# LongmaoTeamTf/deep_recommenders

Hardware: AMD Instinct MI355X
Metric: examples/sec/node DeepFM (26 sparse feats, 10M vocab, dim 64) (higher is better)
Workload: dtype f32; 1 GPU; DeepFM Criteo-shape synthetic training step (BASELINE.json configs[2]): 26 sparse + 13 dense, 10000000 vocab/field hashed on device, dim 64, DNN [256, 32]+[1] relu, sigmoid-CE, fused SGD; batch 65536 per GPU, ids uniform; tables on one GPU (66.6 GB); gemm_split=f16x2, global_batch=65536, parallelism=single, per_kernel_events=False

## Files before the change

deep_recommenders_amd/csrc/bf3_wgrad.hip:

```cpp
#ifndef DR_NT_WGRAD_GATHER
#define DR_NT_WGRAD_GATHER 0
#endif
#include "bf3_rs_core.h"

namespace {

using namespace drrs;

struct TnRsArgs {
    const float* X; int64_t ldx;
    const float* Y; int64_t ldy;
    int64_t R; int32_t F; int32_t N;
    int64_t per; int32_t split;
    float* partial; float* colsum;
    const int32_t* ids_t; const int64_t* row_base; const float* table; int32_t nf; const float* dense_pad;
    const uint32_t* x_amax; const uint32_t* x2_amax; const uint32_t* y_amax;
};

template <int GATHER, int H2 = 0>
__global__ __launch_bounds__(512, 2) void bf3_gemm_tn_rs_kernel(TnRsArgs g) {
    constexpr int NW = 8, BMF = 32 * NW, BN = 256, NT = BN / 32;
    constexpr int NPL = RS_NPL<H2>, B_PLANE = RS_B_PLANE, STAGE = RS_STAGE<H2>;
    __shared__ __attribute__((aligned(1024))) unsigned char smem[2 * STAGE];

    const int tid = threadIdx.x, lane = tid & 63;
    const int wave = __builtin_amdgcn_readfirstlane(tid >> 6);
    const int l31 = lane & 31, hi = lane >> 5;
    const int tiles_n = (g.N + BN - 1) / BN, tiles_f = (g.F + BMF - 1) / BMF;
    const int per_slice = tiles_f * tiles_n;
    const int Fp = tiles_f * BMF, Np = tiles_n * BN;
    const int lid = xcd_remap(blockIdx.x, per_slice * g.split);
    const int slice = lid / per_slice, t = lid % per_slice;
    const int f0 = (t / tiles_n) * BMF, n0 = (t % tiles_n) * BN;
    const int64_t r_begin = (int64_t)slice * g.per;
    int64_t r_end = r_begin + g.per;
    if (r_end > g.R) r_end = g.R;
    const int nk = (int)((r_end - r_begin + BK - 1) / BK);
    const bool want_cs = g.colsum != nullptr && f0 == 0;
    float h2_sx = 1.f, h2_sy = 1.f;
    if constexpr (H2) {
        float inv;
        h2_prologue(g.x_amax, g.x2_amax, g.y_amax, h2_sx, h2_sy, inv);
    }

    const int fcol = min(f0 + wave * 32 + l31, g.F - 1);
    const int ncol = min(n0 + wave * 32 + l31, g.N - 1);
    const unsigned lds0 = (unsigned)(uintptr_t)(lds_ptr_t)smem;
    const int sw = tn_img_swizzle(l31);
    unsigned b_addr[2];
#pragma unroll
    for (int s = 0; s < 2; ++s) b_addr[s] = rs_frag_addr(lds0, l31, hi, sw, s);
    unsigned char* const wrow = smem + (wave * 32 + l31) * 64;

    float xa[16], yb[16];
    const unsigned xoff = (unsigned)((16 * hi * g.ldx + fcol) * 4), yoff = (unsigned)((16 * hi * g.ldy + ncol) * 4);
    auto load_raw = [&](float (&dst)[16], const float* base, int64_t ld, unsigned voff, int64_t r0) {
        if (r0 + BK <= r_end) {
// ... 156 lines not shown
            __builtin_amdgcn_sched_barrier(0);
        }
    }
    float* out = g.partial + ((int64_t)slice * Fp + f0 + wave * 32 + 4 * hi) * Np + n0 + l31;
#pragma unroll
    for (int nt = 0; nt < NT; ++nt)
#pragma unroll
        for (int reg = 0; reg < 16; ++reg) out[(int64_t)((reg & 3) + 8 * (reg >> 2)) * Np + nt * 32] = acc[nt][reg];
    if (want_cs) {
        cs += __shfl_xor(cs, 32, 64);
        if (hi == 0) g.colsum[(int64_t)slice * Np + n0 + wave * 32 + l31] = cs;
    }
}

template <int V>
__global__ __launch_bounds__(64) void bf3_tn_rs_reduce_kernel(const float* __restrict__ partial, const float* __restrict__ colsum,
                                                              int32_t split, int32_t F, int32_t N, int32_t Fp, int32_t Np,
                                                              float scale, float* __restrict__ dst, int64_t ld,
                                                              float* __restrict__ dstb, const uint32_t* __restrict__ x_amax = nullptr,
                                                              const uint32_t* __restrict__ x2_amax = nullptr,
                                                              const uint32_t* __restrict__ y_amax = nullptr) {
    typedef float vec_t __attribute__((ext_vector_type(V)));
    const int f = blockIdx.x;
    const int n = ((int)blockIdx.y * 64 + (int)threadIdx.x) * V;
    if (n >= N) return;
    const int64_t ps = (int64_t)Fp * Np;
    float wscale = scale;
    if (x_amax != nullptr) {
        float sx, ix, sy, iy;
        h2_scale_of(max(x_amax[0], x2_amax != nullptr ? x2_amax[0] : 0u), sx, ix);
        h2_scale_of(y_amax[0], sy, iy);
        wscale = scale * (ix * iy);
    }
    auto sum_slices = [&](const float* p, int64_t stride) -> vec_t {
        vec_t acc = 0.f;
        int s = 0;
        for (; s + 8 <= split; s += 8) {
            vec_t v[8];
#pragma unroll
            for (int u = 0; u < 8; ++u) v[u] = *reinterpret_cast<const vec_t*>(p + (s + u) * stride);
#pragma unroll
            for (int u = 0; u < 8; ++u) acc += v[u];
        }
        for (; s < split; ++s) acc += *reinterpret_cast<const vec_t*>(p + s * stride);
        return acc;
    };
    const vec_t acc = sum_slices(partial + (int64_t)f * Np + n, ps);
    float* d = dst + (int64_t)f * ld + n;
    if (V == 1 || n + V <= N) {
        vec_t o = *reinterpret_cast<vec_t*>(d);
#pragma unroll
        for (int c = 0; c < V; ++c) o[c] = fmaf(wscale, acc[c], o[c]);
        *reinterpret_cast<vec_t*>(d) = o;
    } else {
#pragma unroll
        for (int c = 0; c < V; ++c)
            if (n + c < N) d[c] = fmaf(wscale, acc[c], d[c]);
    }
    if (f == 0 && colsum != nullptr && dstb != nullptr) {
        const vec_t cacc = sum_slices(colsum + n, Np);
#pragma unroll
        for (int c = 0; c < V; ++c)
            if (n + c < N) dstb[n + c] = fmaf(scale, cacc[c], dstb[n + c]);
    }
}

void launch_tn_rs_reduce(const float* partial, const float* colsum, int split, int32_t F, int32_t N, int Fp, int Np, float scale,
                         float* dst, int64_t ld, float* dstb, const uint32_t* x_amax, const uint32_t* x2_amax, const uint32_t* y_amax,
                         dr_stream_t stream) {
    const bool vec = ((reinterpret_cast<uintptr_t>(partial) | reinterpret_cast<uintptr_t>(dst)) & 15) == 0 && (ld & 3) == 0;
    if (vec)
        hipLaunchKernelGGL(bf3_tn_rs_reduce_kernel<4>, dim3(F, (N + 255) / 256), dim3(64), 0, dr_s(stream), partial, colsum, split, F, N,
                           Fp, Np, scale, dst, ld, dstb, x_amax, x2_amax, y_amax);
    else
        hipLaunchKernelGGL(bf3_tn_rs_reduce_kernel<1>, dim3(F, (N + 63) / 64), dim3(64), 0, dr_s(stream), partial, colsum, split, F, N,
                           Fp, Np, scale, dst, ld, dstb, x_amax, x2_amax, y_amax);
}

void tn_rs_plan(int64_t R, int32_t F, int32_t N, int& split, int64_t& per, int& Fp, int& Np) {
    const int tf = (F + 255) / 256, tn = (N + 255) / 256;
    Fp = tf * 256;
    Np = tn * 256;
    int64_t sp = 256 / ((int64_t)tf * tn);
    const int64_t max_split = (R + 16 * BK - 1) / (16 * BK);
    if (sp > max_split) sp = max_split;
    if (sp < 1) sp = 1;
    per = ((R + sp - 1) / sp + BK - 1) / BK * BK;
    split = (int)((R + per - 1) / per);
}
}

extern "C" int64_t dr_bf3_wgrad_workspace_bytes(int64_t R, int32_t F, int32_t N) {
    if (R <= 0 || F <= 0 || N <= 0) return 0;
    int split, Fp, Np;
    int64_t per;
    tn_rs_plan(R, F, N, split, per, Fp, Np);
    return ((int64_t)split * Fp * Np + (int64_t)split * Np) * (int64_t)sizeof(float);
}

static int wgrad_impl(const float* x, int64_t ld_x, const float* dy, int64_t ld_dy, int64_t R, int32_t F, int32_t N,
                      float scale, float* dstW, int64_t ld_w, float* dstb, void* workspace, int64_t workspace_bytes,
                      dr_stream_t stream, const uint32_t* x_amax = nullptr, const uint32_t* dy_amax = nullptr) {
    if (R <= 0 || F <= 0 || N <= 0) return DR_EINVAL;
    if (!x || !dy || !dstW || !workspace || ld_x < F || ld_dy < N || ld_w < N) return DR_EINVAL;
    if (workspace_bytes < dr_bf3_wgrad_workspace_bytes(R, F, N)) return DR_EINVAL;
    int split, Fp, Np;
    int64_t per;
    tn_rs_plan(R, F, N, split, per, Fp, Np);
    float* partial = static_cast<float*>(workspace);
    float* colsum = partial + (int64_t)split * Fp * Np;
    TnRsArgs g{x, ld_x, dy, ld_dy, R, F, N, per, split, partial, dstb != nullptr ? colsum : nullptr, nullptr, nullptr, nullptr, 0, nullptr,
               x_amax, nullptr, dy_amax};
    const int grid = (Fp / 256) * (Np / 256) * split;
    if (x_amax != nullptr) hipLaunchKernelGGL((bf3_gemm_tn_rs_kernel<0, 1>), dim3(grid), dim3(512), 0, dr_s(stream), g);
    else hipLaunchKernelGGL((bf3_gemm_tn_rs_kernel<0, 0>), dim3(grid), dim3(512), 0, dr_s(stream), g);
    launch_tn_rs_reduce(partial, dstb != nullptr ? colsum : nullptr, split, F, N, Fp, Np, scale, dstW, ld_w, dstb, x_amax, nullptr, dy_amax,
                        stream);
    DR_CHECK_LAUNCH();
    return DR_OK;
}

extern "C" int dr_bf3_wgrad(const float* x, int64_t ld_x, const float* dy, int64_t ld_dy, int64_t R, int32_t F, int32_t N,
                            float scale, float* dstW, int64_t ld_w, float* dstb, void* workspace, int64_t workspace_bytes,
                            dr_stream_t stream) {
    return wgrad_impl(x, ld_x, dy, ld_dy, R, F, N, scale, dstW, ld_w, dstb, workspace, workspace_bytes, stream);
}

extern "C" int dr_h2_wgrad(const float* x, int64_t ld_x, const uint32_t* x_amax, const float* dy, int64_t ld_dy, const uint32_t* dy_amax,
                           int64_t R, int32_t F, int32_t N, float scale, float* dstW, int64_t ld_w, float* dstb, void* workspace,
                           int64_t workspace_bytes, dr_stream_t stream) {
    if (!x_amax || !dy_amax) return DR_EINVAL;
    return wgrad_impl(x, ld_x, dy, ld_dy, R, F, N, scale, dstW, ld_w, dstb, workspace, workspace_bytes, stream, x_amax, dy_amax);
}

static int wgrad_emb_impl(const int32_t* ids_t, int64_t R, int32_t nf, const int64_t* row_base, const float* table, int32_t D,
                          const float* dense_pad, const float* dy, int64_t ld_dy, int32_t F, int32_t N, float scale, float* dstW,
                          int64_t ld_w, float* dstb, void* workspace, int64_t workspace_bytes, int32_t parts, dr_stream_t stream,
                          const uint32_t* table_amax = nullptr, const uint32_t* dense_amax = nullptr, const uint32_t* dy_amax = nullptr) {
    if (R <= 0 || F <= 0 || N <= 0 || nf <= 0) return DR_EINVAL;
    if (table_amax != nullptr && (!dy_amax || (F > 64 * nf && !dense_amax))) return DR_EINVAL;
    if (D != 64 || F < 64 * nf || F > 64 * nf + 32) return DR_ESHAPE;
    if (!ids_t || !row_base || !table || !dy || !dstW || !workspace || ld_dy < N || ld_w < N) return DR_EINVAL;
    if (F > 64 * nf && !dense_pad) return DR_EINVAL;
    if (workspace_bytes < dr_bf3_wgrad_workspace_bytes(R, F, N)) return DR_EINVAL;
    int split, Fp, Np;
    int64_t per;
    tn_rs_plan(R, F, N, split, per, Fp, Np);
    float* partial = static_cast<float*>(workspace);
    float* colsum = partial + (int64_t)split * Fp * Np;
    TnRsArgs g{nullptr, 0, dy, ld_dy, R, F, N, per, split, partial, dstb != nullptr ? colsum : nullptr, ids_t, row_base, table, nf,
               F > 64 * nf ? dense_pad : nullptr, table_amax, F > 64 * nf ? dense_amax : nullptr, dy_amax};
    const int grid = (Fp / 256) * (Np / 256) * split;
    if (parts & 1) {
        if (table_amax != nullptr) hipLaunchKernelGGL((bf3_gemm_tn_rs_kernel<1, 1>), dim3(grid), dim3(512), 0, dr_s(stream), g);
        else hipLaunchKernelGGL((bf3_gemm_tn_rs_kernel<1, 0>), dim3(grid), dim3(512), 0, dr_s(stream), g);
    }
    if (parts & 2)
        launch_tn_rs_reduce(partial, dstb != nullptr ? colsum : nullptr, split, F, N, Fp, Np, scale, dstW, ld_w, dstb, table_amax,
                            F > 64 * nf ? dense_amax : nullptr, dy_amax, stream);
    DR_CHECK_LAUNCH();
    return DR_OK;
}

extern "C" int dr_bf3_wgrad_emb(const int32_t* ids_t, int64_t R, int32_t nf, const int64_t* row_base, const float* table, int32_t D,
                                const float* dense_pad, const float* dy, int64_t ld_dy, int32_t F, int32_t N, float scale, float* dstW,
                                int64_t ld_w, float* dstb, void* workspace, int64_t workspace_bytes, int32_t parts, dr_stream_t stream) {
    if (parts < 1 || parts > 3) return DR_EINVAL;
    return wgrad_emb_impl(ids_t, R, nf, row_base, table, D, dense_pad, dy, ld_dy, F, N, scale, dstW, ld_w, dstb, workspace, workspace_bytes,
                          parts, stream);
}

extern "C" int dr_h2_wgrad_emb(const int32_t* ids_t, int64_t R, int32_t nf, const int64_t* row_base, const float* table, int32_t D,
                               const uint32_t* table_amax, const float* dense_pad, const uint32_t* dense_amax, const float* dy, int64_t ld_dy,
                               const uint32_t* dy_amax, int32_t F, int32_t N, float scale, float* dstW, int64_t ld_w, float* dstb,
// ... 6 lines not shown
```

deep_recommenders_amd/csrc/emb_sorted.hip:

```cpp
#include <cstdlib>
#include "dr_common.h"
#include <hip/amd_detail/amd_hip_unsafe_atomics.h>
#include <cstring>

namespace {

constexpr int CH = 32;

#ifndef DR_K4_NT
#define DR_K4_NT 1
#endif
typedef float dr_f4v __attribute__((ext_vector_type(4)));
__device__ __forceinline__ float4 ld4_stream(const float* p) {
#if DR_K4_NT
    const dr_f4v v = __builtin_nontemporal_load(reinterpret_cast<const dr_f4v*>(p));
    return make_float4(v.x, v.y, v.z, v.w);
#else
    return *reinterpret_cast<const float4*>(p);
#endif
}
__device__ __forceinline__ void st4_stream(float* p, const float4 v) {
#if DR_K4_NT
    const dr_f4v w = {v.x, v.y, v.z, v.w};
    __builtin_nontemporal_store(w, reinterpret_cast<dr_f4v*>(p));
// ... 309 lines not shown
template <int LPR, int U, bool ADAM>
__global__ DR_K4_LB void emb_bwd_sorted_kernel(BwdSortedArgs a, AdamArgs ad, int grid_d) {
    if ((int)blockIdx.x < grid_d)
        emb_bwd_dups_body<LPR, ADAM>(blockIdx.x, grid_d, a.rows, a.slots, a.n, a.dup_heads, a.dup_count, a.F, a.D, a.num_rows, a.grad,
                                     a.ld, a.concat, a.ldc, a.sum_x, a.d_fm_logit, a.slot_lin, a.scale, a.table, a.lin_w, ad, a.x_sorted,
                                     a.det != 0, a.amax);
    else if (a.dups_only) {
        if (!ADAM && a.lin_bias != nullptr && a.d_fm_logit != nullptr) dr_block_sum_axpy(a.d_fm_logit, a.B, a.scale, a.lin_bias);
    } else
        emb_bwd_unique_body<LPR, U, ADAM>(blockIdx.x - grid_d, gridDim.x - grid_d, a.ids, a.flags, a.B, a.F, a.row_base, a.D, a.grad,
                                          a.ld, a.concat, a.ldc, a.sum_x, a.d_fm_logit, a.slot_lin, a.scale, a.table,
                                          a.skip_unique_lin ? nullptr : a.lin_w, a.lin_bias, ad, a.lin_old_t, a.amax);
}

template <int LPR>
__global__ __launch_bounds__(256) void emb_bwd_hot_apply_kernel(BwdSortedArgs a) {
    constexpr int NS = DR_WAVE / LPR;
    const int lane = threadIdx.x & 63, grp = lane / LPR, sub = lane % LPR;
    const int D = a.D, F = a.F;
    const bool dvalid = sub < (D >> 2);
    const int subc = dvalid ? sub : (D >> 2) - 1;
    const bool any_lin = a.lin_w != nullptr && (a.d_fm_logit != nullptr || a.slot_lin != nullptr);
    const int64_t nwaves = (int64_t)gridDim.x * (blockDim.x >> 6);
    const int64_t wave0 = (int64_t)blockIdx.x * (blockDim.x >> 6) + (threadIdx.x >> 6);
    const int64_t nheads = a.dup_count[0], n = a.dup_count[1];
    float wmax = 0.f;
    constexpr int SCREEN = 16;
    for (int64_t h0 = wave0 * SCREEN; h0 < nheads; h0 += nwaves * SCREEN) {
        const int64_t h = h0 + lane;
        int64_t my_i = 0, my_stop = 0;
// ... 74 lines not shown
                if (lane == 0) a.lin_w[k] = fmaf(a.scale, dls, a.lin_w[k]);
            }
        }
    }
    if (a.amax != nullptr) amax_commit(a.amax, wmax);
}

}

static int bwd_sorted_impl(const int64_t* ids, const int64_t* row_base, const int64_t* sorted_rows,
                           const int32_t* sorted_slots, const uint8_t* unique_flags, const int32_t* dup_heads,
                           const int32_t* dup_count, int64_t B, int32_t F, int32_t D, int64_t num_rows, const float* grad,
                           int64_t ld_grad, const float* concat, int64_t ld_concat, const float* sum_x,
                           const float* d_fm_logit, const float* slot_lin_grad, float scale, float* dst_table,
                           float* dst_lin, float* dst_bias, const AdamArgs* adam, float* x_sorted, dr_stream_t stream,
                           int parts, const float* lin_old_t, uint32_t* table_amax) {
    if (B < 0 || F <= 0 || F > 64 || D < 4 || D > 256 || (D & 3) || num_rows <= 0) return DR_EINVAL;
    const int64_t n = B * F;
    if (n == 0) return DR_OK;
    if (!ids || !row_base || !sorted_rows || !sorted_slots || !unique_flags || !dup_heads || !dup_count || !grad ||
        !dst_table ||
        ld_grad < (int64_t)F * D || (ld_grad & 3))
        return DR_EINVAL;
    if (concat != nullptr && (ld_concat < (int64_t)F * D || (ld_concat & 3) || sum_x == nullptr)) return DR_EINVAL;
    if (sum_x != nullptr && d_fm_logit == nullptr) return DR_EINVAL;
    if (sum_x != nullptr && concat == nullptr && x_sorted == nullptr) return DR_EINVAL;
    int lpr = 1;
    while (lpr * 4 < D) lpr <<= 1;
    const uint64_t* rows = reinterpret_cast<const uint64_t*>(sorted_rows);
    const int grid_u = dr_grid_for(B, 4, 8192);
    const int grid_d = 2048;
    AdamArgs ad{};
    if (adam != nullptr) ad = *adam;
    static const bool det_on = [] { const char* e = getenv("DR_K4_DETERMINISTIC"); return !(e != nullptr && e[0] == '0'); }();
    const int det = (adam == nullptr && x_sorted != nullptr && det_on) ? 1 : 0;
    const BwdSortedArgs ba{ids, unique_flags, B, F, row_base, D, grad, ld_grad, concat, ld_concat, sum_x, d_fm_logit, slot_lin_grad,
                           scale, dst_table, dst_lin, dst_bias, rows, sorted_slots, n, dup_heads, dup_count, (uint64_t)num_rows,
                           x_sorted, det, (adam == nullptr && (parts & 4)) ? 1 : 0,
                           slot_lin_grad == nullptr ? lin_old_t : nullptr, table_amax, (parts & 8) ? 1 : 0};
#ifdef DR_K4_U
    constexpr int K4_U_OVERRIDE = DR_K4_U;
#else
    constexpr int K4_U_OVERRIDE = 0;
#endif
#define LAUNCH(L, ADAM_)                                                                                              \
    {                                                                                                                 \
        constexpr int NS_ = 64 / L;                                                                                   \
        constexpr int U_ = K4_U_OVERRIDE > 0 ? K4_U_OVERRIDE : (NS_ >= 16 ? 2 : 4);                                   \
        hipLaunchKernelGGL((emb_bwd_sorted_kernel<L, U_, ADAM_>), dim3(grid_d + ((parts & 8) ? 1 : grid_u)), dim3(256), 0, dr_s(stream), ba, ad,    \
                           grid_d);                                                                                   \
    }
#define CALL(L)                                                                                                       \
    if (adam != nullptr) LAUNCH(L, true) else LAUNCH(L, false)
    if (parts & 1)
    switch (lpr) {
        case 1: CALL(1); break;
        case 2: CALL(2); break;
        case 4: CALL(4); break;
        case 8: CALL(8); break;
        case 16: CALL(16); break;
        case 32: CALL(32); break;
        case 64: CALL(64); break;
        default: return DR_EINVAL;
    }
#undef CALL
#undef LAUNCH
// ... 15 lines not shown
    return DR_OK;
}

extern "C" int dr_emb_pool_bwd_sorted(const int64_t* ids, const int64_t* row_base, const int64_t* sorted_rows,
                                      const int32_t* sorted_slots, const uint8_t* unique_flags,
                                      const int32_t* dup_heads, const int32_t* dup_count, int64_t B, int32_t F,
                                      int32_t D, int64_t num_rows, const float* grad, int64_t ld_grad,
                                      const float* concat, int64_t ld_concat, const float* sum_x,
                                      const float* d_fm_logit, const float* slot_lin_grad, float scale,
                                      float* dst_table, float* dst_lin, float* dst_bias, float* x_sorted,
                                      const float* lin_old_t, int32_t parts, uint32_t* table_amax, dr_stream_t stream) {
    if (parts < 1 || parts > 15 || (parts & 3) == 0) return DR_EINVAL;
    return bwd_sorted_impl(ids, row_base, sorted_rows, sorted_slots, unique_flags, dup_heads, dup_count, B, F, D, num_rows,
                           grad, ld_grad, concat, ld_concat, sum_x, d_fm_logit, slot_lin_grad, scale, dst_table, dst_lin,
                           dst_bias, nullptr, x_sorted, stream, parts, lin_old_t, table_amax);
}

namespace {
__global__ __launch_bounds__(256) void lin_update_unique_kernel(const int64_t* __restrict__ ids, const uint8_t* __restrict__ flags,
                                                                int64_t n, int32_t F, const int64_t* __restrict__ row_base,
                                                                const float* __restrict__ d_fm_logit,
                                                                const float* __restrict__ slot_lin, float scale,
                                                                float* __restrict__ lin_w) {
    const int64_t stride = (int64_t)gridDim.x * blockDim.x;
    for (int64_t s = (int64_t)blockIdx.x * blockDim.x + threadIdx.x; s < n; s += stride) {
        const int64_t id = ids[s];
        if (id < 0 || !flags[s]) continue;
        const int64_t b = s / F;
        const int f = (int)(s - b * F);
        const int64_t row = row_base[f] + id;
// ... 215 lines not shown
```

deep_recommenders_amd/engine.py:

```python
import math
import os
from typing import List, Optional, Sequence

import torch

from . import ops
from .ops import _pad4


_SIDE_STREAMS = {}


def _side_streams(device):
    key = str(torch.device(device))
    if key not in _SIDE_STREAMS:
        _SIDE_STREAMS[key] = (torch.cuda.Stream(device=device), torch.cuda.Stream(device=device))
    return _SIDE_STREAMS[key]


class DeepFMEngine:
    def __init__(self, num_fields: int, vocab_per_field: int, dim: int, dnn_units: Sequence[int], batch: int,
                 num_dense: int = 0, lr: float = 0.01, device="cuda", seed: int = 42, hashed: bool = True,
                 table_init_std: Optional[float] = None, lin_init_std: float = 0.0, sorted_bwd: bool = True,
                 optimizer: str = "sgd", beta1: float = 0.9, beta2: float = 0.999, eps: float = 1e-8):
# ... 154 lines not shown
                        and D == 64 and not self.lin_side and self.lin_old_t is not None
                        and self.Ws[0].shape[0] >= F * D)
        _rs = os.environ.get("DR_REDUCE_SIDE", "0")
        self.reduce_side = sorted_bwd and optimizer == "sgd" and _rs in ("1", "2")
        self.reduce_side_wgrad = self.reduce_side and _rs == "1" and not self.h2
        self._small_pending = False
        self._planes_pending = False
        self._planes_pending_l0 = False
        self._k4_fused_done = False
        self._in_train_step = False
        self._early_issued = False
        _ov = os.environ.get("DR_OVERLAP_DW", "0")
        self.overlap_dw = _ov == "1"
        if self.overlap_dw:
            self.no_concat = False
        self.concurrent = {}
        if self.overlap_dw:
            k4 = "emb_pool_bwd_adam" if optimizer == "adam" else "emb_pool_bwd"
            self.concurrent = {"linear_bwd_dw_L0": k4, k4: "linear_bwd_dw_L0"}
            self.side2 = torch.cuda.Stream(device=device)
            self.ev_dx = torch.cuda.Event()
            self.ev_dw = torch.cuda.Event()

    @property
    def dense_pad(self):
        return self._dense_pads[self.cur] if self._dense_pads is not None else None

    @property
    def dense_amax(self):
        return self._dense_amaxs[self.cur] if self._dense_amaxs is not None else None
# ... 143 lines not shown
                tot += max(first.elapsed_time(fa), first.elapsed_time(fb))
            out.append({"kernels": [a, b], "joint_us": tot / n * 1e3})
        return out

    def _wgrad_reduce_deferred(self, i):
        return self.reduce_side_wgrad and i == 0 and self.no_concat and self.wplanes[0] is not None and not self.overlap_dw

    def _side_part2(self, fn):
        self.ev_part1.record()
        with torch.cuda.stream(self.side):
            self.side.wait_event(self.ev_part1)
            fn()
            self.ev_small.record(self.side)
        self._small_pending = True

    def _wgrad(self, i, x, dy, sc, dstW, dstb):
        if i == 0 and self.h2:
            ops.h2_wgrad_emb(self._ids_t[self.cur], self.row_base, self.table, self.tab_amax, self.dense_pad, self.dense_amax, dy,
                             self.dh0_amax, sc, dstW, dstb, workspace=self.wg_ws[0], parts=1 if self._wgrad_reduce_deferred(i) else 3)
        elif i == 0 and self.no_concat:
            ops.bf3_wgrad_emb(self._ids_t[self.cur], self.row_base, self.table, self.dense_pad, dy, sc, dstW, dstb,
                              workspace=self.wg_ws[0], parts=1 if self._wgrad_reduce_deferred(i) else 3)
        elif self.wg_ws[i] is not None:
            ops.bf3_wgrad(x, dy, sc, dstW, dstb, workspace=self.wg_ws[i])
        else:
            ops.linear_bwd_dw(x, dy, sc, dstW, dstb, workspace=self.dw_ws[i])

    def forward(self, keys: torch.Tensor, dense: Optional[torch.Tensor], labels: Optional[torch.Tensor],
                loss_mode: int = ops.LOSS_SIGMOID_CE):
        F, D = self.F, self.D
        B = self.B
        if self.optimizer == "adam":
            self.flat_grads.zero_()
        if self._planes_pending:
# ... 258 lines not shown
                torch.cuda.current_stream().wait_event(self.ev_lin)
            self._prefetch_issue(mark)
        else:
            self._k("emb_pool_bwd", "hbm", self.alg_bytes_bwd(),
                    lambda: ops.emb_pool_bwd(self.ids, F, self.col_start, self.row_base, D, self.d_concat, self.concat,
                                             self.sum_x, self.d_logit, -lr, self.table, self.lin_w, self.lin_bias))
        if self._small_pending:
            torch.cuda.current_stream().wait_event(self.ev_small)
            self._small_pending = False
        if self.overlap_dw and not adam:
            torch.cuda.current_stream().wait_event(self.ev_dw)

    def _backward_l0_fused_k4(self, x, dy, sc, dstW, dstb, fl):
        lr = self.lr
        torch.cuda.current_stream().wait_event(self.ev_sorted)
        self._k("linear_bwd_dw_L0", "mfma", fl, lambda: self._wgrad(0, x, dy, sc, dstW, dstb))
        w_old = self.wplanes[0].w
        early = self._early_issued
        rs = self.side_r if early else self.side
        self._refresh_stream = rs
        self.ev_dw_done.record()
        with torch.cuda.stream(rs):
            rs.wait_event(self.ev_dw_done)
            self.wplanes[0].refresh()
            self.ev_planes.record(rs)
        self._planes_pending = True
        self._planes_pending_l0 = True
        mark = self._prefetch_mark()
        if early:
            self._prefetch_issue(mark)
        if not self._k4_det:
            ops.emb_snapshot_sorted_rows(self.plan, self.table, self.R, self.x_sorted)
        work = self.alg_bytes_bwd() - 4.0 * self.B * self.F * self.D + 4.0 * self.B * dy.shape[1]
        self._k("emb_pool_bwd_fused_dgrad_L0", "hbm", work,
                lambda: ops.h2_dgrad_emb_sgd(dy, self.dh0_amax, w_old, self._ids_t[self.cur], self.plan, self.row_base, self.table,
                                             self.lin_w, self.lin_old_t, self.sum_x, self.d_logit, -lr, self.d_concat, table_amax=self.tab_amax))
        k4 = lambda parts: ops.emb_pool_bwd_sorted(self.ids, self.row_base, self.plan, self.D, self.R, self.d_concat, self.d_logit, -lr,
                                                   self.table, self.lin_w, self.lin_bias, sum_x=self.sum_x, x_sorted=self.x_sorted,
                                                   parts=parts | 8, lin_old_t=self.lin_old_t, table_amax=self.tab_amax)
        self._k("emb_pool_bwd_dups", "hbm", 0, lambda: k4(1))
        self._k("emb_hot_rows_apply", "hbm", 0, lambda: k4(2))
        if not early:
            self._prefetch_issue(mark)
        self._k4_fused_done = True

    def _launch_sort(self):
        self.ev_ids.record()
        with torch.cuda.stream(self.side):
            self.side.wait_event(self.ev_ids)
            self._k("emb_sort_slots(side stream, overlapped)", "overlap", self.B * self.F * 36,
                    lambda: ops.emb_sort_slots(self.ids, self.row_base, self.R, self.plan))
            self.ev_sorted.record(self.side)

    def _adam_finish(self):
        self.t += 1
# ... 78 lines not shown
```

deep_recommenders_amd/ops.py:

```python
from typing import Optional, Sequence

import torch

from . import _lib
from ._lib import check, lib, ptr, stream_ptr


def _c(t: torch.Tensor, dtype) -> torch.Tensor:
    if t.dtype != dtype:
        raise TypeError("expected %s, got %s" % (dtype, t.dtype))
    return t if t.is_contiguous() else t.contiguous()


def hash_bucket_i64(keys: torch.Tensor, col_buckets: torch.Tensor, out: Optional[torch.Tensor] = None):
    keys = _c(keys, torch.int64)
    B, C = keys.shape
    col_buckets = _c(col_buckets, torch.int64)
    assert col_buckets.numel() == C
    if out is None:
        out = torch.empty_like(keys)
    check(lib().dr_hash_bucket_i64(ptr(keys), B, C, ptr(col_buckets), ptr(out), stream_ptr()), "dr_hash_bucket_i64")
    return out


# ... 533 lines not shown
    return out


def emb_pool_bwd_sorted(ids, row_base, plan, D, num_rows, grad, d_fm_logit, scale, dst_table, dst_lin=None, dst_bias=None,
                        concat=None, sum_x=None, slot_lin_grad=None, x_sorted=None, parts=3, lin_old_t=None, table_amax=None):
    ids = _c(ids, torch.int64)
    B, F = ids.shape
    assert grad.stride(1) == 1
    assert lin_old_t is None or (lin_old_t.shape == (F, B) and lin_old_t.is_contiguous() and lin_old_t.dtype == torch.float32)
    check(lib().dr_emb_pool_bwd_sorted(ptr(ids), ptr(row_base), ptr(plan.rows), ptr(plan.slots), ptr(plan.flags),
                                       ptr(plan.dup_heads), ptr(plan.dup_count), B, F, D, int(num_rows), ptr(grad),
                                       grad.stride(0), ptr(concat), concat.stride(0) if concat is not None else 0,
                                       ptr(sum_x), ptr(d_fm_logit), ptr(slot_lin_grad), float(scale), ptr(dst_table), ptr(dst_lin),
                                       ptr(dst_bias), ptr(x_sorted), ptr(lin_old_t), int(parts), ptr(table_amax), stream_ptr()),
          "dr_emb_pool_bwd_sorted")


def h2_dgrad_emb_sgd(dy, dy_amax, w: "H2Planes", ids_t, plan, row_base, table, lin_w, lin_old_t, sum_x, d_fm_logit, scale, d_concat,
                     table_amax=None):
    F, M = ids_t.shape
    K = dy.shape[1]
    assert dy.stride(1) == 1 and d_concat.stride(1) == 1 and table.is_contiguous() and table.shape[1] == 64 and sum_x.is_contiguous()
    assert ids_t.dtype == torch.int32 and ids_t.is_contiguous() and dy.shape[0] == M and w.rows >= 64 * F
    assert (lin_w is None) == (lin_old_t is None)
    assert lin_old_t is None or (lin_old_t.shape == (F, M) and lin_old_t.is_contiguous())
    check(lib().dr_h2_dgrad_emb_sgd(ptr(dy), dy.stride(0), ptr(dy_amax), ptr(w.buf), w.plane_stride, w.ld, ptr(w.amax), M, F, K,
                                    ptr(ids_t), ptr(plan.flags), ptr(row_base), ptr(table), ptr(lin_w), ptr(lin_old_t), ptr(sum_x),
                                    ptr(d_fm_logit), float(scale), ptr(d_concat), d_concat.stride(0), ptr(table_amax), stream_ptr()),
          "dr_h2_dgrad_emb_sgd")

# ... 2217 lines not shown
```

include/dr_hotpath.h:

```cpp
#ifndef DR_HOTPATH_H
#define DR_HOTPATH_H

#include <stdint.h>

#ifdef __cplusplus
extern "C" {
#endif

#define DR_OK 0
#define DR_EINVAL (-1)
#define DR_ELAUNCH (-2)
#define DR_ESHAPE (-3)

typedef void* dr_stream_t;

const char* dr_version(void);

#define DR_GEMM_BF16X3 0
#define DR_GEMM_NATIVE_F32 1
int32_t dr_set_gemm_mode(int32_t mode);
int32_t dr_get_gemm_mode(void);

#define DR_GEMM_SPLIT_BF16X3 0
#define DR_GEMM_SPLIT_F16X2 1
// ... 277 lines not shown
                              const float* dense_pad, const uint32_t* dense_amax, float* concat, int64_t ld_concat, int32_t K,
                              const void* wt_planes, int64_t plane_stride, int64_t ld_planes, const uint32_t* w_amax, int32_t N,
                              const float* bias, int32_t act, float* sum_x, float* fm_logit, float* out, int64_t ld_out,
                              float* lin_vals_t, const float* W1, int64_t ld_w1, const float* b1, int32_t H, const float* w2,
                              int64_t ld_w2, const float* b2, const float* labels, int32_t loss_mode, float scale, float* dst_w1,
                              int64_t ld_dst_w1, float* dst_b1, float* dst_w2, int64_t ld_dst_w2, float* dst_b2, float* prob,
                              float* d_logit, float* d_h, int64_t ld_dh, float* dx, int64_t ld_dx, float* loss_out, void* workspace,
                              int64_t workspace_bytes, int32_t parts, uint32_t* dx_amax, dr_stream_t stream);
int dr_h2_wgrad(const float* x, int64_t ld_x, const uint32_t* x_amax, const float* dy, int64_t ld_dy, const uint32_t* dy_amax, int64_t R,
                int32_t F, int32_t N, float scale, float* dstW, int64_t ld_w, float* dstb, void* workspace, int64_t workspace_bytes,
                dr_stream_t stream);
int dr_h2_wgrad_emb(const int32_t* ids_t, int64_t R, int32_t nf, const int64_t* row_base, const float* table, int32_t D,
                    const uint32_t* table_amax, const float* dense_pad, const uint32_t* dense_amax, const float* dy, int64_t ld_dy,
                    const uint32_t* dy_amax, int32_t F, int32_t N, float scale, float* dstW, int64_t ld_w, float* dstb, void* workspace,
                    int64_t workspace_bytes, int32_t parts, dr_stream_t stream);


int dr_cin_fwd(const float* x0, const float* x, int64_t B, int32_t H0, int32_t Hk, int32_t D, const float* W,
               int32_t Fm, const float* bias, int32_t act, float* out, dr_stream_t stream);
int dr_cin_bwd(const float* x0, const float* x, int64_t B, int32_t H0, int32_t Hk, int32_t D, const float* W,
               int32_t Fm, int32_t act, const float* out, const float* d_out, float* d_x0, float* d_x, float* dW,
               float* dbias, dr_stream_t stream);

int dr_cin_pool_fwd(const float* x0, const float* x, int64_t B, int32_t H0, int32_t Hk, int32_t D, const float* W, int32_t Fm,
                    const float* bias, int32_t act, float* out, float* pooled, dr_stream_t stream);
int64_t dr_cin_pool_bwd_workspace_bytes(int64_t B, int32_t H0, int32_t Hk, int32_t D, int32_t Fm);
int dr_cin_pool_bwd(const float* x0, const float* x, int64_t B, int32_t H0, int32_t Hk, int32_t D, const float* W, int32_t Fm,
                    int32_t act, const float* out, const float* d_out, const float* d_pooled, float* d_x0, int32_t accumulate_x0,
                    float* d_x, float* dW, float* dbias, void* ws, int64_t ws_bytes, dr_stream_t stream);

// ... 176 lines not shown
```

Measured before the change: 70.79 million examples/sec.

## Fold wgrad split-K reduce into embedding dups backward kernel as rider blocks

The layer-0 weight-gradient split-K reduction no longer runs as its own kernel. It is appended as extra rider blocks to the embedding duplicate-row backward kernel, which removes a launch and lets the two memory-bound phases overlap. The GEMM kernel now writes the amax scale values into a workspace header, so the reduce no longer depends on amax buffers that the embedding update may mutate. The plane refresh is moved to after the fused kernel. This adds coupling and raises the risk of ordering bugs between the table amax update and the reduce scaling.

```diff
diff --git a/deep_recommenders_amd/csrc/bf3_wgrad.hip b/deep_recommenders_amd/csrc/bf3_wgrad.hip
--- a/deep_recommenders_amd/csrc/bf3_wgrad.hip
+++ b/deep_recommenders_amd/csrc/bf3_wgrad.hip
@@ -2,6 +2,7 @@
 #define DR_NT_WGRAD_GATHER 0
 #endif
 #include "bf3_rs_core.h"
+#include "tn_rs_reduce.h"
 
 namespace {
 
@@ -15,6 +16,7 @@
     float* partial; float* colsum;
     const int32_t* ids_t; const int64_t* row_base; const float* table; int32_t nf; const float* dense_pad;
     const uint32_t* x_amax; const uint32_t* x2_amax; const uint32_t* y_amax;
+    uint32_t* hdr;
 };
 
 template <int GATHER, int H2 = 0>
@@ -41,6 +43,10 @@
     if constexpr (H2) {
         float inv;
         h2_prologue(g.x_amax, g.x2_amax, g.y_amax, h2_sx, h2_sy, inv);
+        if (lid == 0 && tid == 0) {
+            g.hdr[0] = max(g.x_amax[0], g.x2_amax != nullptr ? g.x2_amax[0] : 0u);
+            g.hdr[1] = g.y_amax[0];
+        }
     }
 
     const int fcol = min(f0 + wave * 32 + l31, g.F - 1);
@@ -227,70 +233,18 @@
 }
 
 template <int V>
-__global__ __launch_bounds__(64) void bf3_tn_rs_reduce_kernel(const float* __restrict__ partial, const float* __restrict__ colsum,
-                                                              int32_t split, int32_t F, int32_t N, int32_t Fp, int32_t Np,
-                                                              float scale, float* __restrict__ dst, int64_t ld,
-                                                              float* __restrict__ dstb, const uint32_t* __restrict__ x_amax = nullptr,
-                                                              const uint32_t* __restrict__ x2_amax = nullptr,
-                                                              const uint32_t* __restrict__ y_amax = nullptr) {
-    typedef float vec_t __attribute__((ext_vector_type(V)));
-    const int f = blockIdx.x;
-    const int n = ((int)blockIdx.y * 64 + (int)threadIdx.x) * V;
-    if (n >= N) return;
-    const int64_t ps = (int64_t)Fp * Np;
-    float wscale = scale;
-    if (x_amax != nullptr) {
-        float sx, ix, sy, iy;
-        h2_scale_of(max(x_amax[0], x2_amax != nullptr ? x2_amax[0] : 0u), sx, ix);
-        h2_scale_of(y_amax[0], sy, iy);
-        wscale = scale * (ix * iy);
-    }
-    auto sum_slices = [&](const float* p, int64_t stride) -> vec_t {
-        vec_t acc = 0.f;
-        int s = 0;
-        for (; s + 8 <= split; s += 8) {
-            vec_t v[8];
-#pragma unroll
-            for (int u = 0; u < 8; ++u) v[u] = *reinterpret_cast<const vec_t*>(p + (s + u) * stride);
-#pragma unroll
-            for (int u = 0; u < 8; ++u) acc += v[u];
-        }
-        for (; s < split; ++s) acc += *reinterpret_cast<const vec_t*>(p + s * stride);
-        return acc;
-    };
-    const vec_t acc = sum_slices(partial + (int64_t)f * Np + n, ps);
-    float* d = dst + (int64_t)f * ld + n;
-    if (V == 1 || n + V <= N) {
-        vec_t o = *reinterpret_cast<vec_t*>(d);
-#pragma unroll
-        for (int c = 0; c < V; ++c) o[c] = fmaf(wscale, acc[c], o[c]);
-        *reinterpret_cast<vec_t*>(d) = o;
-    } else {
-#pragma unroll
-        for (int c = 0; c < V; ++c)
-            if (n + c < N) d[c] = fmaf(wscale, acc[c], d[c]);
-    }
-    if (f == 0 && colsum != nullptr && dstb != nullptr) {
-        const vec_t cacc = sum_slices(colsum + n, Np);
-#pragma unroll
-        for (int c = 0; c < V; ++c)
-            if (n + c < N) dstb[n + c] = fmaf(scale, cacc[c], dstb[n + c]);
-    }
-}
-
-void launch_tn_rs_reduce(const float* partial, const float* colsum, int split, int32_t F, int32_t N, int Fp, int Np, float scale,
-                         float* dst, int64_t ld, float* dstb, const uint32_t* x_amax, const uint32_t* x2_amax, const uint32_t* y_amax,
-                         dr_stream_t stream) {
-    const bool vec = ((reinterpret_cast<uintptr_t>(partial) | reinterpret_cast<uintptr_t>(dst)) & 15) == 0 && (ld & 3) == 0;
-    if (vec)
-        hipLaunchKernelGGL(bf3_tn_rs_reduce_kernel<4>, dim3(F, (N + 255) / 256), dim3(64), 0, dr_s(stream), partial, colsum, split, F, N,
-                           Fp, Np, scale, dst, ld, dstb, x_amax, x2_amax, y_amax);
-    else
-        hipLaunchKernelGGL(bf3_tn_rs_reduce_kernel<1>, dim3(F, (N + 63) / 64), dim3(64), 0, dr_s(stream), partial, colsum, split, F, N,
-                           Fp, Np, scale, dst, ld, dstb, x_amax, x2_amax, y_amax);
-}
-
-void tn_rs_plan(int64_t R, int32_t F, int32_t N, int& split, int64_t& per, int& Fp, int& Np) {
+__global__ __launch_bounds__(TN_RS_RED_THREADS) void bf3_tn_rs_reduce_kernel(TnRsApply a) {
+    tn_rs_reduce_block<V>(a, blockIdx.x, threadIdx.x);
+}
+
+void launch_tn_rs_reduce(const TnRsApply& a, dr_stream_t stream) {
+    const int nlb = tn_rs_reduce_blocks(a.F, a.N, a.vec);
+    if (a.vec) hipLaunchKernelGGL(bf3_tn_rs_reduce_kernel<4>, dim3(nlb), dim3(TN_RS_RED_THREADS), 0, dr_s(stream), a);
+    else hipLaunchKernelGGL(bf3_tn_rs_reduce_kernel<1>, dim3(nlb), dim3(TN_RS_RED_THREADS), 0, dr_s(stream), a);
+}
+}
+
+void drrs::tn_rs_plan(int64_t R, int32_t F, int32_t N, int& split, int64_t& per, int& Fp, int& Np) {
     const int tf = (F + 255) / 256, tn = (N + 255) / 256;
     Fp = tf * 256;
     Np = tn * 256;
@@ -301,14 +255,13 @@
     per = ((R + sp - 1) / sp + BK - 1) / BK * BK;
     split = (int)((R + per - 1) / per);
 }
-}
 
 extern "C" int64_t dr_bf3_wgrad_workspace_bytes(int64_t R, int32_t F, int32_t N) {
     if (R <= 0 || F <= 0 || N <= 0) return 0;
     int split, Fp, Np;
     int64_t per;
     tn_rs_plan(R, F, N, split, per, Fp, Np);
-    return ((int64_t)split * Fp * Np + (int64_t)split * Np) * (int64_t)sizeof(float);
+    return ((int64_t)split * Fp * Np + (int64_t)split * Np + TN_RS_HDR_WORDS) * (int64_t)sizeof(float);
 }
 
 static int wgrad_impl(const float* x, int64_t ld_x, const float* dy, int64_t ld_dy, int64_t R, int32_t F, int32_t N,
@@ -320,15 +273,14 @@
     int split, Fp, Np;
     int64_t per;
     tn_rs_plan(R, F, N, split, per, Fp, Np);
-    float* partial = static_cast<float*>(workspace);
-    float* colsum = partial + (int64_t)split * Fp * Np;
-    TnRsArgs g{x, ld_x, dy, ld_dy, R, F, N, per, split, partial, dstb != nullptr ? colsum : nullptr, nullptr, nullptr, nullptr, 0, nullptr,
-               x_amax, nullptr, dy_amax};
+    const bool h2 = x_amax != nullptr;
+    const TnRsApply ap = tn_rs_apply_of(workspace, split, F, N, Fp, Np, h2, scale, dstW, ld_w, dstb);
+    TnRsArgs g{x, ld_x, dy, ld_dy, R, F, N, per, split, const_cast<float*>(ap.partial), const_cast<float*>(ap.colsum), nullptr, nullptr, nullptr, 0,
+               nullptr, x_amax, nullptr, dy_amax, const_cast<uint32_t*>(ap.hdr)};
     const int grid = (Fp / 256) * (Np / 256) * split;
-    if (x_amax != nullptr) hipLaunchKernelGGL((bf3_gemm_tn_rs_kernel<0, 1>), dim3(grid), dim3(512), 0, dr_s(stream), g);
+    if (h2) hipLaunchKernelGGL((bf3_gemm_tn_rs_kernel<0, 1>), dim3(grid), dim3(512), 0, dr_s(stream), g);
     else hipLaunchKernelGGL((bf3_gemm_tn_rs_kernel<0, 0>), dim3(grid), dim3(512), 0, dr_s(stream), g);
-    launch_tn_rs_reduce(partial, dstb != nullptr ? colsum : nullptr, split, F, N, Fp, Np, scale, dstW, ld_w, dstb, x_amax, nullptr, dy_amax,
-                        stream);
+    launch_tn_rs_reduce(ap, stream);
     DR_CHECK_LAUNCH();
     return DR_OK;
 }
@@ -359,18 +311,16 @@
     int split, Fp, Np;
     int64_t per;
     tn_rs_plan(R, F, N, split, per, Fp, Np);
-    float* partial = static_cast<float*>(workspace);
-    float* colsum = partial + (int64_t)split * Fp * Np;
-    TnRsArgs g{nullptr, 0, dy, ld_dy, R, F, N, per, split, partial, dstb != nullptr ? colsum : nullptr, ids_t, row_base, table, nf,
-               F > 64 * nf ? dense_pad : nullptr, table_amax, F > 64 * nf ? dense_amax : nullptr, dy_amax};
+    const bool h2 = table_amax != nullptr;
+    const TnRsApply ap = tn_rs_apply_of(workspace, split, F, N, Fp, Np, h2, scale, dstW, ld_w, dstb);
+    TnRsArgs g{nullptr, 0, dy, ld_dy, R, F, N, per, split, const_cast<float*>(ap.partial), const_cast<float*>(ap.colsum), ids_t, row_base, table,
+               nf, F > 64 * nf ? dense_pad : nullptr, table_amax, F > 64 * nf ? dense_amax : nullptr, dy_amax, const_cast<uint32_t*>(ap.hdr)};
     const int grid = (Fp / 256) * (Np / 256) * split;
     if (parts & 1) {
-        if (table_amax != nullptr) hipLaunchKernelGGL((bf3_gemm_tn_rs_kernel<1, 1>), dim3(grid), dim3(512), 0, dr_s(stream), g);
+        if (h2) hipLaunchKernelGGL((bf3_gemm_tn_rs_kernel<1, 1>), dim3(grid), dim3(512), 0, dr_s(stream), g);
         else hipLaunchKernelGGL((bf3_gemm_tn_rs_kernel<1, 0>), dim3(grid), dim3(512), 0, dr_s(stream), g);
     }
-    if (parts & 2)
-        launch_tn_rs_reduce(partial, dstb != nullptr ? colsum : nullptr, split, F, N, Fp, Np, scale, dstW, ld_w, dstb, table_amax,
-                            F > 64 * nf ? dense_amax : nullptr, dy_amax, stream);
+    if (parts & 2) launch_tn_rs_reduce(ap, stream);
     DR_CHECK_LAUNCH();
     return DR_OK;
 }
diff --git a/deep_recommenders_amd/csrc/emb_sorted.hip b/deep_recommenders_amd/csrc/emb_sorted.hip
--- a/deep_recommenders_amd/csrc/emb_sorted.hip
+++ b/deep_recommenders_amd/csrc/emb_sorted.hip
@@ -1,5 +1,6 @@
 #include <cstdlib>
 #include "dr_common.h"
+#include "tn_rs_reduce.h"
 #include <hip/amd_detail/amd_hip_unsafe_atomics.h>
 #include <cstring>
 
@@ -347,6 +348,19 @@
 }
 
 template <int LPR>
+__global__ __launch_bounds__(256) void emb_bwd_dups_apply_kernel(BwdSortedArgs a, drrs::TnRsApply ap, int grid_d) {
+    const int bid = blockIdx.x;
+    if (bid < grid_d)
+        emb_bwd_dups_body<LPR, false>(bid, grid_d, a.rows, a.slots, a.n, a.dup_heads, a.dup_count, a.F, a.D, a.num_rows, a.grad, a.ld,
+                                      a.concat, a.ldc, a.sum_x, a.d_fm_logit, a.slot_lin, a.scale, a.table, a.lin_w, AdamArgs{}, a.x_sorted,
+                                      a.det != 0, a.amax);
+    else if (bid == grid_d) {
+        if (a.lin_bias != nullptr && a.d_fm_logit != nullptr) dr_block_sum_axpy(a.d_fm_logit, a.B, a.scale, a.lin_bias);
+    } else
+        drrs::tn_rs_reduce_ride(ap, bid - grid_d - 1, (int)gridDim.x - grid_d - 1, threadIdx.x);
+}
+
+template <int LPR>
 __global__ __launch_bounds__(256) void emb_bwd_hot_apply_kernel(BwdSortedArgs a) {
     constexpr int NS = DR_WAVE / LPR;
     const int lane = threadIdx.x & 63, grp = lane / LPR, sub = lane % LPR;
@@ -451,7 +465,7 @@
                            int64_t ld_grad, const float* concat, int64_t ld_concat, const float* sum_x,
                            const float* d_fm_logit, const float* slot_lin_grad, float scale, float* dst_table,
                            float* dst_lin, float* dst_bias, const AdamArgs* adam, float* x_sorted, dr_stream_t stream,
-                           int parts, const float* lin_old_t, uint32_t* table_amax) {
+                           int parts, const float* lin_old_t, uint32_t* table_amax, const drrs::TnRsApply* apply = nullptr) {
     if (B < 0 || F <= 0 || F > 64 || D < 4 || D > 256 || (D & 3) || num_rows <= 0) return DR_EINVAL;
     const int64_t n = B * F;
     if (n == 0) return DR_OK;
@@ -480,13 +494,17 @@
 #else
     constexpr int K4_U_OVERRIDE = 0;
 #endif
+    const int nlb = apply != nullptr ? drrs::tn_rs_reduce_blocks(apply->F, apply->N, apply->vec) : 0;
+    const int riders = nlb < 1024 ? nlb : 1024;
 #define LAUNCH(L, ADAM_)                                                                                              \
-    {                                                                                                                 \
+    { if (apply != nullptr) {                                                                                         \
+        hipLaunchKernelGGL((emb_bwd_dups_apply_kernel<L>), dim3(grid_d + 1 + riders), dim3(256), 0, dr_s(stream), ba, *apply, grid_d);     \
+    } else {                                                                                                          \
         constexpr int NS_ = 64 / L;                                                                                   \
         constexpr int U_ = K4_U_OVERRIDE > 0 ? K4_U_OVERRIDE : (NS_ >= 16 ? 2 : 4);                                   \
         hipLaunchKernelGGL((emb_bwd_sorted_kernel<L, U_, ADAM_>), dim3(grid_d + ((parts & 8) ? 1 : grid_u)), dim3(256), 0, dr_s(stream), ba, ad,    \
                            grid_d);                                                                                   \
-    }
+    } }
 #define CALL(L)                                                                                                       \
     if (adam != nullptr) LAUNCH(L, true) else LAUNCH(L, false)
     if (parts & 1)
@@ -532,6 +550,27 @@
     return bwd_sorted_impl(ids, row_base, sorted_rows, sorted_slots, unique_flags, dup_heads, dup_count, B, F, D, num_rows,
                            grad, ld_grad, concat, ld_concat, sum_x, d_fm_logit, slot_lin_grad, scale, dst_table, dst_lin,
                            dst_bias, nullptr, x_sorted, stream, parts, lin_old_t, table_amax);
+}
+
+extern "C" int dr_emb_pool_bwd_dups_apply(const int64_t* ids, const int64_t* row_base, const int64_t* sorted_rows,
+                                          const int32_t* sorted_slots, const uint8_t* unique_flags, const int32_t* dup_heads,
+                                          const int32_t* dup_count, int64_t B, int32_t F, int32_t D, int64_t num_rows, const float* grad,
+                                          int64_t ld_grad, const float* sum_x, const float* d_fm_logit, float scale, float* dst_table,
+                                          float* dst_lin, float* dst_bias, float* x_sorted, const float* lin_old_t, int32_t parts,
+                                          uint32_t* table_amax, void* wg_workspace, int64_t wg_workspace_bytes, int64_t wg_R, int32_t wg_F,
+                                          int32_t wg_N, int32_t wg_h2, float wg_scale, float* dstW, int64_t ld_w, float* dstb,
+                                          dr_stream_t stream) {
+    if (parts != 9 && parts != 11) return DR_EINVAL;
+    if (wg_R <= 0 || wg_F <= 0 || wg_N <= 0 || !wg_workspace || !dstW || ld_w < wg_N) return DR_EINVAL;
+    if (wg_workspace_bytes < dr_bf3_wgrad_workspace_bytes(wg_R, wg_F, wg_N)) return DR_EINVAL;
+    if (B <= 0) return DR_EINVAL;
+    int split, Fp, Np;
+    int64_t per;
+    drrs::tn_rs_plan(wg_R, wg_F, wg_N, split, per, Fp, Np);
+    const drrs::TnRsApply ap = drrs::tn_rs_apply_of(wg_workspace, split, wg_F, wg_N, Fp, Np, wg_h2 != 0, wg_scale, dstW, ld_w, dstb);
+    return bwd_sorted_impl(ids, row_base, sorted_rows, sorted_slots, unique_flags, dup_heads, dup_count, B, F, D, num_rows, grad, ld_grad,
+                           nullptr, 0, sum_x, d_fm_logit, nullptr, scale, dst_table, dst_lin, dst_bias, nullptr, x_sorted, stream, parts,
+                           lin_old_t, table_amax, &ap);
 }
 
 namespace {
diff --git a/deep_recommenders_amd/csrc/tn_rs_reduce.h b/deep_recommenders_amd/csrc/tn_rs_reduce.h
--- /dev/null
+++ b/deep_recommenders_amd/csrc/tn_rs_reduce.h
@@ -0,0 +1,92 @@
+#pragma once
+#include "rs_args.h"
+
+namespace drrs {
+
+constexpr int TN_RS_HDR_WORDS = 4;
+constexpr int TN_RS_RED_THREADS = 256;
+
+struct TnRsApply {
+    const float* partial; const float* colsum;
+    const uint32_t* hdr;
+    int32_t split, F, N, Fp, Np;
+    float scale;
+    float* dst; int64_t ld; float* dstb;
+    int32_t vec;
+};
+
+__host__ __device__ inline int tn_rs_reduce_blocks(int F, int N, int vec) {
+    const int w = vec ? (N + 3) / 4 : N;
+    return (int)(((int64_t)F * w + TN_RS_RED_THREADS - 1) / TN_RS_RED_THREADS);
+}
+
+template <int V>
+__device__ __forceinline__ void tn_rs_reduce_block(const TnRsApply& a, int lb, int tid) {
+    typedef float vec_t __attribute__((ext_vector_type(V)));
+    const int w = (a.N + V - 1) / V;
+    const int64_t t = (int64_t)lb * TN_RS_RED_THREADS + tid;
+    const int f = (int)(t / w);
+    const int n = (int)(t - (int64_t)f * w) * V;
+    if (f >= a.F) return;
+    const int split = a.split, N = a.N, Np = a.Np;
+    const int64_t ps = (int64_t)a.Fp * Np;
+    float wscale = a.scale;
+    if (a.hdr != nullptr) {
+        float sx, ix, sy, iy;
+        h2_scale_of(a.hdr[0], sx, ix);
+        h2_scale_of(a.hdr[1], sy, iy);
+        wscale = a.scale * (ix * iy);
+    }
+    auto sum_slices = [&](const float* p, int64_t stride) -> vec_t {
+        vec_t acc = 0.f;
+        int s = 0;
+        for (; s + 8 <= split; s += 8) {
+            vec_t v[8];
+#pragma unroll
+            for (int u = 0; u < 8; ++u) v[u] = *reinterpret_cast<const vec_t*>(p + (s + u) * stride);
+#pragma unroll
+            for (int u = 0; u < 8; ++u) acc += v[u];
+        }
+        for (; s < split; ++s) acc += *reinterpret_cast<const vec_t*>(p + s * stride);
+        return acc;
+    };
+    const vec_t acc = sum_slices(a.partial + (int64_t)f * Np + n, ps);
+    float* d = a.dst + (int64_t)f * a.ld + n;
+    if (V == 1 || n + V <= N) {
+        vec_t o = *reinterpret_cast<vec_t*>(d);
+#pragma unroll
+        for (int c = 0; c < V; ++c) o[c] = fmaf(wscale, acc[c], o[c]);
+        *reinterpret_cast<vec_t*>(d) = o;
+    } else {
+#pragma unroll
+        for (int c = 0; c < V; ++c)
+            if (n + c < N) d[c] = fmaf(wscale, acc[c], d[c]);
+    }
+    if (f == 0 && a.colsum != nullptr && a.dstb != nullptr) {
+        const vec_t cacc = sum_slices(a.colsum + n, Np);
+#pragma unroll
+        for (int c = 0; c < V; ++c)
+            if (n + c < N) a.dstb[n + c] = fmaf(a.scale, cacc[c], a.dstb[n + c]);
+    }
+}
+
+__device__ __forceinline__ void tn_rs_reduce_ride(const TnRsApply& a, int rider, int nriders, int tid) {
+    const int nlb = tn_rs_reduce_blocks(a.F, a.N, a.vec);
+    for (int lb = rider; lb < nlb; lb += nriders) {
+        if (a.vec) tn_rs_reduce_block<4>(a, lb, tid);
+        else tn_rs_reduce_block<1>(a, lb, tid);
+    }
+}
+
+inline TnRsApply tn_rs_apply_of(void* workspace, int split, int32_t F, int32_t N, int Fp, int Np, bool h2, float scale, float* dst,
+                                int64_t ld, float* dstb) {
+    float* partial = static_cast<float*>(workspace);
+    float* colsum = partial + (int64_t)split * Fp * Np;
+    const uint32_t* hdr = reinterpret_cast<const uint32_t*>(colsum + (int64_t)split * Np);
+    const bool vec = ((reinterpret_cast<uintptr_t>(partial) | reinterpret_cast<uintptr_t>(dst)) & 15) == 0 && (ld & 3) == 0;
+    return TnRsApply{partial, dstb != nullptr ? colsum : nullptr, h2 ? hdr : nullptr, split, F, N, Fp, Np, scale, dst, ld, dstb, vec ? 1 : 0};
+}
+
+void tn_rs_plan(int64_t R, int32_t F, int32_t N, int& split, int64_t& per, int& Fp, int& Np);
+
+}
diff --git a/deep_recommenders_amd/engine.py b/deep_recommenders_amd/engine.py
--- a/deep_recommenders_amd/engine.py
+++ b/deep_recommenders_amd/engine.py
@@ -192,6 +192,8 @@
         self.overlap_dw = _ov == "1"
         if self.overlap_dw:
             self.no_concat = False
+        self.fold_reduces = (os.environ.get("DR_FOLD_REDUCES", "1") != "0" and self.tail_in_fwd and self.fuse_k4 and self.h2
+                             and optimizer == "sgd" and not self.overlap_dw and not self.reduce_side)
         self.concurrent = {}
         if self.overlap_dw:
             k4 = "emb_pool_bwd_adam" if optimizer == "adam" else "emb_pool_bwd"
@@ -365,10 +367,11 @@
             self.ev_small.record(self.side)
         self._small_pending = True
 
-    def _wgrad(self, i, x, dy, sc, dstW, dstb):
+    def _wgrad(self, i, x, dy, sc, dstW, dstb, main_only=False):
         if i == 0 and self.h2:
             ops.h2_wgrad_emb(self._ids_t[self.cur], self.row_base, self.table, self.tab_amax, self.dense_pad, self.dense_amax, dy,
-                             self.dh0_amax, sc, dstW, dstb, workspace=self.wg_ws[0], parts=1 if self._wgrad_reduce_deferred(i) else 3)
+                             self.dh0_amax, sc, dstW, dstb, workspace=self.wg_ws[0],
+                             parts=1 if (main_only or self._wgrad_reduce_deferred(i)) else 3)
         elif i == 0 and self.no_concat:
             ops.bf3_wgrad_emb(self._ids_t[self.cur], self.row_base, self.table, self.dense_pad, dy, sc, dstW, dstb,
                               workspace=self.wg_ws[0], parts=1 if self._wgrad_reduce_deferred(i) else 3)
@@ -657,18 +660,24 @@
     def _backward_l0_fused_k4(self, x, dy, sc, dstW, dstb, fl):
         lr = self.lr
         torch.cuda.current_stream().wait_event(self.ev_sorted)
-        self._k("linear_bwd_dw_L0", "mfma", fl, lambda: self._wgrad(0, x, dy, sc, dstW, dstb))
+        fold = self.fold_reduces
+        self._k("linear_bwd_dw_L0", "mfma", fl, lambda: self._wgrad(0, x, dy, sc, dstW, dstb, main_only=fold))
         w_old = self.wplanes[0].w
         early = self._early_issued
-        rs = self.side_r if early else self.side
-        self._refresh_stream = rs
-        self.ev_dw_done.record()
-        with torch.cuda.stream(rs):
-            rs.wait_event(self.ev_dw_done)
-            self.wplanes[0].refresh()
-            self.ev_planes.record(rs)
-        self._planes_pending = True
-        self._planes_pending_l0 = True
+        rs = self.side_r if (early or fold) else self.side
+
+        def refresh_planes_behind():
+            self._refresh_stream = rs
+            self.ev_dw_done.record()
+            with torch.cuda.stream(rs):
+                rs.wait_event(self.ev_dw_done)
+                self.wplanes[0].refresh()
+                self.ev_planes.record(rs)
+            self._planes_pending = True
+            self._planes_pending_l0 = True
+
+        if not fold:
+            refresh_planes_behind()
         mark = self._prefetch_mark()
         if early:
             self._prefetch_issue(mark)
@@ -681,7 +690,14 @@
         k4 = lambda parts: ops.emb_pool_bwd_sorted(self.ids, self.row_base, self.plan, self.D, self.R, self.d_concat, self.d_logit, -lr,
                                                    self.table, self.lin_w, self.lin_bias, sum_x=self.sum_x, x_sorted=self.x_sorted,
                                                    parts=parts | 8, lin_old_t=self.lin_old_t, table_amax=self.tab_amax)
-        self._k("emb_pool_bwd_dups", "hbm", 0, lambda: k4(1))
+        if fold:
+            self._k("emb_pool_bwd_dups", "hbm", 0,
+                    lambda: ops.emb_pool_bwd_dups_apply(self.ids, self.row_base, self.plan, self.D, self.R, self.d_concat, self.d_logit, -lr,
+                                                        self.table, self.lin_w, self.lin_bias, self.sum_x, self.x_sorted, self.lin_old_t,
+                                                        self.tab_amax, self.wg_ws[0], self.B, sc, dstW, dstb, wg_h2=True, parts=1))
+            refresh_planes_behind()
+        else:
+            self._k("emb_pool_bwd_dups", "hbm", 0, lambda: k4(1))
         self._k("emb_hot_rows_apply", "hbm", 0, lambda: k4(2))
         if not early:
             self._prefetch_issue(mark)
diff --git a/deep_recommenders_amd/ops.py b/deep_recommenders_amd/ops.py
--- a/deep_recommenders_amd/ops.py
+++ b/deep_recommenders_amd/ops.py
@@ -571,6 +571,21 @@
                                        ptr(sum_x), ptr(d_fm_logit), ptr(slot_lin_grad), float(scale), ptr(dst_table), ptr(dst_lin),
                                        ptr(dst_bias), ptr(x_sorted), ptr(lin_old_t), int(parts), ptr(table_amax), stream_ptr()),
           "dr_emb_pool_bwd_sorted")
+
+
+def emb_pool_bwd_dups_apply(ids, row_base, plan, D, num_rows, grad, d_fm_logit, scale, dst_table, dst_lin, dst_bias, sum_x, x_sorted,
+                            lin_old_t, table_amax, wg_workspace, wg_R, wg_scale, dstW, dstb=None, wg_h2=True, parts=1):
+    ids = _c(ids, torch.int64)
+    B, F = ids.shape
+    wg_F, wg_N = dstW.shape
+    assert grad.stride(1) == 1 and dstW.stride(1) == 1
+    assert lin_old_t is None or (lin_old_t.shape == (F, B) and lin_old_t.is_contiguous() and lin_old_t.dtype == torch.float32)
+    check(lib().dr_emb_pool_bwd_dups_apply(ptr(ids), ptr(row_base), ptr(plan.rows), ptr(plan.slots), ptr(plan.flags), ptr(plan.dup_heads),
+                                           ptr(plan.dup_count), B, F, D, int(num_rows), ptr(grad), grad.stride(0), ptr(sum_x),
+                                           ptr(d_fm_logit), float(scale), ptr(dst_table), ptr(dst_lin), ptr(dst_bias), ptr(x_sorted),
+                                           ptr(lin_old_t), int(parts) | 8, ptr(table_amax), ptr(wg_workspace), wg_workspace.numel() * 4,
+                                           int(wg_R), wg_F, wg_N, 1 if wg_h2 else 0, float(wg_scale), ptr(dstW), dstW.stride(0), ptr(dstb),
+                                           stream_ptr()), "dr_emb_pool_bwd_dups_apply")
 
 
 def h2_dgrad_emb_sgd(dy, dy_amax, w: "H2Planes", ids_t, plan, row_base, table, lin_w, lin_old_t, sum_x, d_fm_logit, scale, d_concat,
diff --git a/include/dr_hotpath.h b/include/dr_hotpath.h
--- a/include/dr_hotpath.h
+++ b/include/dr_hotpath.h
@@ -315,6 +315,13 @@
                     const uint32_t* table_amax, const float* dense_pad, const uint32_t* dense_amax, const float* dy, int64_t ld_dy,
                     const uint32_t* dy_amax, int32_t F, int32_t N, float scale, float* dstW, int64_t ld_w, float* dstb, void* workspace,
                     int64_t workspace_bytes, int32_t parts, dr_stream_t stream);
+int dr_emb_pool_bwd_dups_apply(const int64_t* ids, const int64_t* row_base, const int64_t* sorted_rows, const int32_t* sorted_slots,
+                               const uint8_t* unique_flags, const int32_t* dup_heads, const int32_t* dup_count, int64_t B, int32_t F,
+                               int32_t D, int64_t num_rows, const float* grad, int64_t ld_grad, const float* sum_x,
+                               const float* d_fm_logit, float scale, float* dst_table, float* dst_lin, float* dst_bias, float* x_sorted,
+                               const float* lin_old_t, int32_t parts, uint32_t* table_amax, void* wg_workspace,
+                               int64_t wg_workspace_bytes, int64_t wg_R, int32_t wg_F, int32_t wg_N, int32_t wg_h2, float wg_scale,
+                               float* dstW, int64_t ld_w, float* dstb, dr_stream_t stream);
 
 
 int dr_cin_fwd(const float* x0, const float* x, int64_t B, int32_t H0, int32_t Hk, int32_t D, const float* W,
```

Measured after the change: 71.59 million examples/sec, median of 6. 1.1% higher.
